# ThatRedox/ChunkyClPlugin

Measured on AMD Instinct MI355X. Metric: Msamples/s, 32x32-chunk scene @1920x1080, higher is better.
Workload: dtype f32

## Files before the change

### chunkyclplugin_amd/csrc/path_state.hpp

```cpp
#pragma once
#include <hip/hip_runtime.h>

#include "kernels.hpp"
#include "rt_device.hpp"

namespace chunky {

struct LdsStack {
    int* base;
    int stride;
    DEV void push(int slot, int v) { base[slot * stride] = v; }
    DEV int pop(int slot) { return base[slot * stride]; }
};
template <int TREE>
DEV void leaf_lookup(const SceneView& S, int bx, int by, int bz, int& data, int& level, int& kind, bool inside = true, int* entry = nullptr) {
    if (TREE < 16 && !inside) bx = by = bz = 0;
    if (TREE == 0) {
        const int* __restrict__ tree = S.octree;
        level = S.octree_depth;
        data = tree[0];
        while (data > 0) {
            level--;
            data = tree[data + ((((bx >> level) & 1) << 2) | (((by >> level) & 1) << 1) | ((bz >> level) & 1))];
        }
// ... 169 lines not shown
    const int sb = i / kSubBlock, px = i % kSubBlock;
    const int x = (bx << kTileLog) + (sb % (kTileEdge / kSubW)) * kSubW + px % kSubW,
              y = (by << kTileLog) + (sb / (kTileEdge / kSubW)) * kSubH + px / kSubW;
    return (x < width && y < height) ? y * width + x : width * height;
}
DEV unsigned fast_quotient(unsigned n, FastDiv f) { return f.m ? __umulhi(n, f.m) >> f.s : n; }

struct SlotPixel {
    int gid, x, y;
};
DEV SlotPixel pool_slot_pixel(const ShardView& T, int width, int height, int slot, FastDiv by_bw) {
    if (T.world != 1 && T.tile != 0) {
        const int gid = slot < T.n_local ? shard_gid(T, slot) : width * height;
        return SlotPixel{gid, gid % width, gid / width};
    }
    const int bw = (width + kTileEdge - 1) >> kTileLog;
    int b = slot >> (2 * kTileLog);
    const int i = slot & (kSampleTile - 1);
    if (T.world != 1) {
        b = b * T.world + T.rank;
        if (b >= bw * ((height + kTileEdge - 1) >> kTileLog)) return SlotPixel{width * height, 0, 0};
    }
    const int by = (int)fast_quotient((unsigned)b, by_bw), bx = b - by * bw;
    const int sb = i / kSubBlock, px = i % kSubBlock;
    const int x = (bx << kTileLog) + (sb % (kTileEdge / kSubW)) * kSubW + px % kSubW,
              y = (by << kTileLog) + (sb / (kTileEdge / kSubW)) * kSubH + px / kSubW;
    return SlotPixel{(x < width && y < height) ? y * width + x : width * height, x, y};
}
__host__ __device__ inline long long pool_tiles(const ShardView& T, int width, int height) {
    if (T.world != 1) return ((long long)T.n_local + kSampleTile - 1) / kSampleTile;
    return (long long)((width + kTileEdge - 1) >> kTileLog) * ((height + kTileEdge - 1) >> kTileLog);
}
DEV int count_lanes(bool p) { return (int)__builtin_popcountll(__ballot(p)); }
enum : int {
    ST_MARCH = 0, ST_BLOCK = 1, ST_SHADE = 2,
    ST_MODEL = 6,
    ST_BVH = 9,
    ST_LEAF = 11,
    ST_TRACED = 10,
    ST_DONE = 3,
    ST_NEXT = 4,
    ST_SETUP = 5,
    ST_IDLE = 7,
    ST_START = 8
};

struct LaneState {
    int gid;
    int sidx;
    unsigned pass : 8;
    unsigned slot : 1;
    unsigned serial : 23;
    f3 mean;
    unsigned rng;
    f3 radiance, throughput, o, d;
    unsigned depth : 8;
    unsigned shadow : 1;
    unsigned oct_hit : 1;
    unsigned trace_hit : 1;
    unsigned cand_level : 4;
    unsigned bvh_which : 1;
    f3 inv;
    float dist_march;
    int steps;
    int cand_data;
    int bvh_cur;
    int bvh_top;
    const int* bvh_base;
    int bvh_head;
    float bvh_dist;
    f3 far;
    int pid;
    unsigned tkind : 2;
    unsigned after_nee : 1;
    f3 pend;
    Hit h;
};

DEV int floor_to_int(float x) {
    int r;
    asm("v_cvt_flr_i32_f32 %0, %1" : "=v"(r) : "v"(x));
    return r;
}

template <bool GUARD = true>
DEV float leaf_exit_distance(const LaneState& L, f3 far, f3 po, int bx, int by, int bz, int level) {
    const int keep = -1 << level;
    const float size = __builtin_ldexpf(1.0f, level);
    const float x0 = (float)(bx & keep), y0 = (float)(by & keep), z0 = (float)(bz & keep);
    float tx = (rt_fma(far.x, size, x0) - po.x) * L.inv.x, ty = (rt_fma(far.y, size, y0) - po.y) * L.inv.y, tz = (rt_fma(far.z, size, z0) - po.z) * L.inv.z;
    if (GUARD) {
        tx = rt_fmax(tx, -rt_inf());
        ty = rt_fmax(ty, -rt_inf());
        tz = rt_fmax(tz, -rt_inf());
    }
    return rt_fmin(tx, rt_fmin(ty, tz));
}
DEV f3 far_of(const f3& inv) { return mk3(inv.x > 0 ? 1.0f : 0.0f, inv.y > 0 ? 1.0f : 0.0f, inv.z > 0 ? 1.0f : 0.0f); }

template <int TREE, bool FARREG = true>
DEV void leaf_exit(const SceneView& S, LaneState& L, f3 po, int bx, int by, int bz, int level) {
    L.dist_march += leaf_exit_distance(L, FARREG ? L.far : far_of(L.inv), po, bx, by, bz, level) + kOffset;
    L.steps += 1;
}

template <int END, bool FARREG = true>
DEV int trace_setup(const SceneView& S, LaneState& L) {
    const int depth = S.octree_depth;
    L.inv = rcp3(L.d);
    if (FARREG) L.far = far_of(L.inv);
    L.dist_march = 0;
    L.steps = 0;
    L.oct_hit = false;
    int lx = (int)rt_floor(L.o.x) >> depth, ly = (int)rt_floor(L.o.y) >> depth, lz = (int)rt_floor(L.o.z) >> depth;
    if ((lx != 0) | (ly != 0) | (lz != 0)) {
        float size = (float)(1 << depth);
        float dist = box_quick(0, size, 0, size, 0, size, L.o, L.inv);
        if (dist != dist || dist < 0) return END;
        L.dist_march += dist + kOffset;
    }
    return ST_MARCH;
}

typedef unsigned long long LaneMask;
DEV bool in_mask(LaneMask m) { return __builtin_amdgcn_inverse_ballot_w64(m); }

DEV unsigned world_edge(const SceneView& S) {
    unsigned edge = 1u << S.octree_depth;
    asm("" : "+s"(edge));
    return edge;
}
template <int TREE, bool GUARD = true>
DEV void march_step(const SceneView& S, const RenderOpts& O, LaneState& L, LaneMask marching, LaneMask& cand_out,
                    LaneMask& live_out, int& data, int& level, const unsigned edge, const LaneMask* far_masks = nullptr, int* entry = nullptr) {
    f3 pos = L.o + L.d * L.dist_march;
    f3 po = pos + L.d * kOffset;
    int bx = floor_to_int(po.x), by = floor_to_int(po.y), bz = floor_to_int(po.z);
    const bool inside = (unsigned)(bx | by | bz) < edge;
    const LaneMask live = marching & __ballot(L.steps < O.draw_depth) & __ballot(!(L.dist_march > L.h.distance)) & __ballot(inside);
    int kind;
    leaf_lookup<TREE>(S, bx, by, bz, data, level, kind, inside, entry);
    const LaneMask hittable = __ballot(kind < 2);
    const LaneMask cand = live & hittable, go = live & ~hittable;
    const f3 far = far_masks ? mk3(in_mask(far_masks[0]) ? 1.0f : 0.0f, in_mask(far_masks[1]) ? 1.0f : 0.0f, in_mask(far_masks[2]) ? 1.0f : 0.0f)
                             : L.far;
    const float step = leaf_exit_distance<GUARD>(L, far, po, bx, by, bz, level) + kOffset;
    const bool advance = in_mask(go);
    L.dist_march = advance ? L.dist_march + step : L.dist_march;
    asm("v_addc_co_u32_e64 %0, vcc, 0, %0, %1" : "+v"(L.steps) : "s"(go) : "vcc");
    cand_out = cand;
    live_out = live;
}

template <int TREE, int END, bool FARREG = true, int KINDS = kBlockAny>
DEV int block_phase(const SceneView& S, LaneState& L) {
    f3 pos = L.o + L.d * L.dist_march;
    f3 po = pos + L.d * kOffset;
    int bx = (int)rt_floor(po.x), by = (int)rt_floor(po.y), bz = (int)rt_floor(po.z);
    Hit t = L.h;
    float dist = block_hit<KINDS>(S, L.cand_data, bx, by, bz, pos, L.d, L.inv, t);
    if (!L.shadow) {
        L.h.normal = t.normal;
        L.h.color = t.color;
        L.h.emittance = t.emittance;
        L.h.spec = t.spec;
    }
    if (dist == dist) {
        if (!L.shadow) {
            L.h.distance = L.dist_march + dist;
            L.h.material = L.cand_data;
        }
        L.oct_hit = true;
        return END;
    }
    leaf_exit<TREE, FARREG>(S, L, po, bx, by, bz, L.cand_level);
    return ST_MARCH;
}
struct WorkQueue {
    int* next;
};
struct WaveArgs {
    SceneView S;
    CameraView C;
    RenderOpts O;
    ShardView T;
    PassSeeds P;
    WorkQueue Q;
    float* res;
    unsigned long long* stats;
    unsigned stack_bytes;
    float* staging;
    unsigned n_samples;
    unsigned xcd_stripe;
    FastDiv div_sub;
    FastDiv div_bw;
    const int* seeds_dev;
};
static_assert(sizeof(WaveArgs) <= 4096, "launch arguments must fit the 4 KB kernel-argument segment");
typedef const WaveArgs __attribute__((address_space(4))) * WaveArgPtr;

template <typename T>
DEV T arg_copy(const T __attribute__((address_space(4))) * p) {
#if defined(__HIP_DEVICE_COMPILE__)
    return *p;
#else
    (void)p;
    return T{};
#endif
}

DEV WaveArgPtr fresh_args() {
    WaveArgPtr a = (WaveArgPtr)__builtin_amdgcn_kernarg_segment_ptr();
    asm volatile("" : "+s"(a));
    return a;
}

struct PartTimers {
    unsigned long long t[10];
    unsigned long long last;
};
enum : int { PT_SKY = 0, PT_SAMPLING, PT_SETUP, PT_DEPOSIT, PT_FOLD, PT_OPEN, PT_HANDOUT, PT_NEWSAMPLE };
template <bool ON>
DEV void part_begin(PartTimers* pt) {
    if (ON) pt->last = __builtin_amdgcn_s_memtime();
}
template <bool ON>
DEV void part_end(PartTimers* pt, int which) {
    if (ON) {
        const unsigned long long now = __builtin_amdgcn_s_memtime();
        pt->t[which] += now - pt->last;
        pt->last = now;
    }
}

template <int TREE, bool BVH, bool PROF = false>
DEV int shade_phase(const SceneView& S, const RenderOpts& O, LaneState& L, LdsStack& stack, PartTimers* pt = nullptr) {
    part_begin<PROF>(pt);
    const bool hit = BVH ? L.trace_hit : L.oct_hit;
    const bool main_trace = !L.shadow;
    if (!hit) {
        const float e = main_trace ? 1.0f : rt_fabs(dot(L.d, L.h.normal));
        L.radiance = L.radiance + sky_radiance(S, L.d, L.throughput, e);
    }
    part_end<PROF>(pt, PT_SKY);
    bool finished = !hit && main_trace;
    bool to_sun = false;
    if (finished) {
    } else if (main_trace) {
        L.o = L.o + L.d * (L.h.distance - kOffset);
        f3 c = mk3(L.h.color.x, L.h.color.y, L.h.color.z);
        L.throughput = L.throughput * c;
        L.radiance = L.radiance + (c * (L.h.emittance * O.emitter_scale)) * L.throughput;
        if (S.sun_flags & 1) to_sun = true;
    } else {
        L.shadow = false;
    }
    if (!finished) {
        const float x1 = rt_pcg_float(&L.rng), x2 = rt_pcg_float(&L.rng);
        float sn, cs;
        rt_sincos(2 * RT_PI_F * x2, &sn, &cs);
        const float cos_a = 1 - x1 + x1 * S.sun_radius_cos;
        const float root = rt_sqrt(to_sun ? 1 - cos_a * cos_a : x1);
        const f3 n = L.h.normal;
        f3 a;
        float len2;
        if (to_sun) {
            const f3 u = S.su * (cs * root), v = S.sv * (sn * root), w = S.sw * cos_a;
            a = (u * v) + w;
            len2 = dot(a, a);
        } else {
            float xx, xy, xz = 0;
            if ((double)rt_fabs(n.x) > 0.1) {
                xx = 0;
                xy = 1;
            } else {
                xx = 1;
                xy = 0;
            }
            a = mk3(xy * n.z - xz * n.y, xz * n.x - xx * n.z, xx * n.y - xy * n.x);
            len2 = a.x * a.x + a.y * a.y + a.z * a.z;
        }
        const float rl = 1 / rt_sqrt(len2);
        a = a * rl;
        if (to_sun) {
            L.d = a;
            L.shadow = true;
        } else {
            const float tx = root * cs, ty = root * sn, tz = rt_sqrt(1 - x1);
            const float vx = a.y * n.z - a.z * n.y, vy = a.z * n.x - a.x * n.z, vz = a.x * n.y - a.y * n.x;
            L.d = f3{a.x * tx + vx * ty + n.x * tz, a.y * tx + vy * ty + n.y * tz, a.z * tx + vz * ty + n.z * tz};
            L.o = L.o + L.d * kOffset;
            L.depth += 1;
            L.h.distance = rt_inf();
            finished = !(L.depth < O.max_depth);
        }
    }
    part_end<PROF>(pt, PT_SAMPLING);
    return finished ? ST_NEXT : ST_SETUP;
}

DEV f3 cosine_direction(f3 n, float x1, float x2) {
    float r = rt_sqrt(x1);
    float theta = 2 * RT_PI_F * x2;
    float st, ct;
    rt_sincos(theta, &st, &ct);
    float tx = r * ct, ty = r * st, tz = rt_sqrt(1 - x1);
    float xx, xy, xz = 0;
    if ((double)rt_fabs(n.x) > 0.1) {
        xx = 0;
        xy = 1;
    } else {
// ... 42 lines not shown
```

### chunkyclplugin_amd/csrc/pool_kernel.inc

```
template <int TREE, int K, bool STATS, bool BVH = false, bool EXT = false, bool SORT = false>
__global__ void __launch_bounds__(256, ((STATS || EXT) ? 4 : (BVH ? CHUNKY_POOL_BVH_WAVES : CHUNKY_POOL_WAVES))) render_pool(WaveArgs unused_by_name) {
    constexpr int WORDS = EXT ? 9 : (BVH ? 8 : CHUNKY_POOL_WORDS);
    constexpr int END = BVH ? ST_TRACED : ST_SHADE;
    constexpr bool SPLIT = SORT;
    static_assert(!SORT || (TREE != 0 && !BVH && !EXT), "sorted block tests: the plain kernel on the re-laid-out tree only");
    extern __shared__ int lds[];
    const int lane = (int)(threadIdx.x & 63u), wave = (int)(threadIdx.x >> 6);
    PoolLds P{nullptr, nullptr, nullptr};
    PathStacks stacks{nullptr, 64 + K};
    {
        const unsigned depth = BVH ? fresh_args()->stack_bytes : 0u;
        char* base = (char*)lds + wave * (K * 16 * WORDS + K * 8 + (64 + K) * depth * 4);
        P.park = (uint4*)base;
        P.tags = (int*)(base + K * 16 * WORDS);
        P.list = P.tags + K;
        stacks.base = (int*)(base + K * 16 * WORDS + K * 8);
        if (lane < K) P.park[lane] = make_uint4(0u, 0u, kFreshDepth | (WORDS <= 7 ? 0u : (unsigned)(64 + lane) << 16), 0u);
    }
    LdsStack stack{lds, 0};
    LaneState L;
    L.h.material = 0;
    L.h.normal = mk3(0, 0, 0);
    L.h.color = f4{0, 0, 0, 0};
    L.h.emittance = 0;
    L.h.distance = 0;
    L.cand_data = 0;
    L.cand_level = 0;
    L.pass = 0;
    L.gid = -1;
    L.sidx = 0;
    L.pid = lane;
    L.tkind = 0;
    L.after_nee = false;
    L.pend = mk3(0, 0, 0);
    L.h.spec = 0;
    L.mean = mk3(0, 0, 0);
    L.slot = 0;
    L.serial = 0;
    L.steps = 0;
    L.rng = 0;
    L.depth = kFreshDepth;
    L.shadow = false;
    L.dist_march = 0;
    L.radiance = mk3(0, 0, 0);
    L.throughput = mk3(0, 0, 0);
    L.o = L.d = L.inv = L.far = mk3(0, 0, 0);
    L.oct_hit = false;
    L.trace_hit = false;
    L.bvh_cur = L.bvh_top = L.bvh_which = L.bvh_head = 0;
    L.bvh_base = nullptr;
    L.bvh_dist = 0;
    unsigned long long prof[9] = {0, 0, 0, 0, 0, 0, 0, 0, 0};
    unsigned long long swap_rounds = 0, swapped = 0;
    PartTimers parts{{0, 0, 0, 0, 0, 0, 0, 0, 0, 0}, 0};
    unsigned long long t_begin = 0;
    if (STATS) t_begin = __builtin_amdgcn_s_memtime();
    XcdClaim claim{xcd_first_range(), 0u, 0u};
    int ranges_tried = 0;
    int st = ST_SHADE;
    int ptag = lane < K ? ST_SHADE : ST_DONE;
    wave_lds_fence();
    int c_march = 0, c_block = 0, c_shade = 0, c_bvh = 0, c_leaf = 0, c_model = 0;
    int model_age = 0;
    auto census = [&]() {
        if (BVH && __ballot(st == ST_TRACED)) {
            const SceneView S = arg_copy(&fresh_args()->S);
            if (st == ST_TRACED) st = rbvh_begin(S, L);
        }
        c_march = count_lanes(st == ST_MARCH) + count_lanes(ptag == ST_MARCH);
        c_block = count_lanes(st == ST_BLOCK) + count_lanes(ptag == ST_BLOCK);
        c_shade = count_lanes(st == ST_SHADE) + count_lanes(ptag == ST_SHADE);
        c_model = SPLIT ? count_lanes(st == ST_MODEL) + count_lanes(ptag == ST_MODEL) : 0;
        c_bvh = BVH ? count_lanes(st == ST_BVH) + count_lanes(ptag == ST_BVH) : 0;
        c_leaf = BVH ? count_lanes(st == ST_LEAF) + count_lanes(ptag == ST_LEAF) : 0;
    };
    census();
    while ((c_march | c_block | c_shade | c_bvh | c_leaf | c_model) != 0) {
        const int v_march = (c_march < 64 ? c_march : 64) * kWMarch, v_block = (c_block < 64 ? c_block : 64) * kWBlock,
                  v_shade = (c_shade < 64 ? c_shade : 64) * kWShade;
        int X = (int)((unsigned)(v_march - v_block - 1) >> 31);
        int v_best = v_block > v_march ? v_block : v_march;
        if (v_shade >= v_best) {
            X = 2;
            v_best = v_shade;
        }
        if (SPLIT) {
            const int v_model = (c_model < 64 ? c_model : 64) * kWModel;
            model_age += 1;
            if (v_model > v_best || c_model * model_age >= kModelFire) {
                X = ST_MODEL;
                v_best = v_model > v_best ? v_model : v_best;
                model_age = 0;
            }
        }
        if (BVH) {
            const int c_walk = c_bvh + c_leaf;
            const int v_walk = (c_walk < 64 ? c_walk : 64) * kWWalk;
            if (v_walk > v_best) { X = 5; v_best = v_walk; }
        }
        unsigned long long t0 = 0;
        if (STATS) t0 = __builtin_amdgcn_s_memtime();
        if (K > 0) {
            const int n = pool_swap<K, WORDS>(P, L, st, ptag, X, lane);
            if (STATS && n) {
                swap_rounds += 1;
                swapped += (unsigned long long)n;
            }
        }
        if (STATS) {
            parts.t[PT_FOLD] += __builtin_amdgcn_s_memtime() - t0;
            parts.t[PT_OPEN] += 1;
            parts.t[PT_HANDOUT] += X == 0 ? 1 : 0;
        }
        int n_exec = 0;
        if (X == 0) {
            WaveArgPtr A = fresh_args();
            const SceneView Sm = arg_copy(&A->S);
            const RenderOpts Om = arg_copy(&A->O);
            const LaneMask entered = __ballot(st == ST_MARCH);
            int nm = __popcll(entered);
            n_exec = nm;
            const int parked_march = c_march - nm;
            const int other_b = c_block < 64 ? c_block : 64, other_s = c_shade < 64 ? c_shade : 64;
            int other = other_b > other_s ? other_b : other_s;
            if (SPLIT) {
                const int other_m = c_model < 64 ? c_model : 64;
                other = other > other_m ? other : other_m;
            }
            int stay = (other + nm + 1) >> 1;
            if (parked_march < kStayFewParked) stay -= BVH ? kStayLongerBvh : kStayLonger;
            if (K > 0 && parked_march >= kPoolRefill && stay < 65 - kPoolRefill) stay = 65 - kPoolRefill;
            if (stay < 1) stay = 1;
            LaneMask marching = entered, to_block = 0;
            L.far = far_of(L.inv);
            const LaneMask* far_masks = nullptr;
            int data, level, entry = 0;
            const float ninf = -rt_inf();
            const bool guard = ((__ballot(L.inv.x == ninf) | __ballot(L.inv.y == ninf) | __ballot(L.inv.z == ninf)) & entered) != 0;
            if (guard)
                march_loop<TREE, true, STATS>(Sm, Om, L, marching, to_block, data, level, nm, stay, far_masks, prof, SPLIT ? &entry : nullptr);
            else
                march_loop<TREE, false, STATS>(Sm, Om, L, marching, to_block, data, level, nm, stay, far_masks, prof, SPLIT ? &entry : nullptr);
            const bool found = in_mask(to_block);
            L.cand_data = found ? data : L.cand_data;
            L.cand_level = found ? level : L.cand_level;
            const int st_found = SPLIT && (entry & 0x2000000) ? ST_MODEL : ST_BLOCK;
            st = found ? st_found : (in_mask(entered & ~marching & ~to_block) ? END : st);
            if (STATS) {
                prof[0] -= 1;
                prof[1] -= (unsigned long long)n_exec;
            }
        } else if (X == 1) {
            n_exec = count_lanes(st == ST_BLOCK);
            const SceneView S = arg_copy(&fresh_args()->S);
            if (st == ST_BLOCK) {
                st = block_phase<TREE, END, false, SPLIT ? kBlockCubes : kBlockAny>(S, L);
                if (WORDS == 6 && st == END) hit_to_march_registers(L);
            }
        } else if (SPLIT && X == ST_MODEL) {
            n_exec = count_lanes(st == ST_MODEL);
            if (STATS) parts.t[8] += (unsigned long long)n_exec + (1ull << 40);
            const SceneView S = arg_copy(&fresh_args()->S);
            asm volatile("; chunky-mark models");
            if (st == ST_MODEL) {
                st = block_phase<TREE, END, false, kBlockModels>(S, L);
                if (WORDS == 6 && st == END) hit_to_march_registers(L);
            }
            asm volatile("; chunky-mark models-end");
        } else if (BVH && X == 5) {
            const SceneView S = arg_copy(&fresh_args()->S);
            int nw = count_lanes(st == ST_BVH);
            n_exec = nw;
            const int parked_walk = c_bvh + c_leaf - nw;
            int stay = nw - kWalkLeave + 1;
            if (K > 0 && parked_walk > 0) {
                const int refill = parked_walk < kWalkLeave ? parked_walk : kWalkLeave;
                if (stay < 65 - refill) stay = 65 - refill;
            }
            if (stay < 1) stay = 1;
            do {
                if (STATS) {
                    prof[3] += 1;
                    prof[4] += (unsigned long long)nw;
                }
                if (st == ST_BVH) st = rwalk_step(S, L, stacks);
                nw = count_lanes(st == ST_BVH);
            } while (nw >= stay);
            if (STATS) {
                prof[3] -= 1;
                prof[4] -= (unsigned long long)n_exec;
            }
        } else {
            n_exec = count_lanes(st == ST_SHADE);
            WaveArgPtr A = fresh_args();
            const SceneView S = arg_copy(&A->S);
            const RenderOpts O = arg_copy(&A->O);
            const bool served = st == ST_SHADE;
            bool fresh = served && L.depth == kFreshDepth;
            if (served && !fresh) {
                if (WORDS == 6) march_registers_to_hit(L);
                st = EXT ? shade_phase_ext<TREE, BVH>(S, O, L) : shade_phase<TREE, BVH, STATS>(S, O, L, stack, &parts);
            }
            part_begin<STATS>(&parts);
            if (st == ST_NEXT) {
                float* __restrict__ out = A->staging + 3 * (size_t)(unsigned)L.sidx;
#if CHUNKY_STAGING_STORE == 1
                out[0] = L.radiance.x, out[1] = L.radiance.y, out[2] = L.radiance.z;
#elif CHUNKY_STAGING_STORE == 2
                __hip_atomic_store(out, L.radiance.x, __ATOMIC_RELAXED, __HIP_MEMORY_SCOPE_AGENT);
                __hip_atomic_store(out + 1, L.radiance.y, __ATOMIC_RELAXED, __HIP_MEMORY_SCOPE_AGENT);
                __hip_atomic_store(out + 2, L.radiance.z, __ATOMIC_RELAXED, __HIP_MEMORY_SCOPE_AGENT);
#elif CHUNKY_STAGING_STORE == 3
                __hip_atomic_store(out, L.radiance.x, __ATOMIC_RELAXED, __HIP_MEMORY_SCOPE_SYSTEM);
                __hip_atomic_store(out + 1, L.radiance.y, __ATOMIC_RELAXED, __HIP_MEMORY_SCOPE_SYSTEM);
                __hip_atomic_store(out + 2, L.radiance.z, __ATOMIC_RELAXED, __HIP_MEMORY_SCOPE_SYSTEM);
#else
                __builtin_nontemporal_store(L.radiance.x, out);
                __builtin_nontemporal_store(L.radiance.y, out + 1);
                __builtin_nontemporal_store(L.radiance.z, out + 2);
#endif
                fresh = true;
            }
            part_end<STATS>(&parts, PT_DEPOSIT);
            const bool need = fresh;
            const unsigned sidx = xcd_claim(A->Q.next + kXcdCounters, claim, ranges_tried, need, A->xcd_stripe, A->n_samples);
            if (need && sidx != kClaimNone) {
                const unsigned n_samples = A->n_samples;
                if (sidx >= n_samples) {
                    st = ST_DONE;
                    fresh = false;
                } else {
                    const CameraView C = arg_copy(&A->C);
                    const ShardView T = arg_copy(&A->T);
                    const unsigned per_sub = (unsigned)A->P.n * (unsigned)kSubBlock;
                    const unsigned sub = fast_quotient(sidx, arg_copy(&A->div_sub)), rem = sidx - sub * per_sub;
                    const unsigned pass = rem / (unsigned)kSubBlock;
                    const int slot = (int)(sub * (unsigned)kSubBlock + (rem & (unsigned)(kSubBlock - 1)));
                    const SlotPixel px = pool_slot_pixel(T, C.width, C.height, slot, arg_copy(&A->div_bw));
                    const int gid = px.gid;
                    if (gid < C.width * C.height) {
                        const int* seeds_dev = A->seeds_dev;
                        const unsigned seed = (unsigned)(seeds_dev ? seeds_dev[pass] : A->P.seed[pass]);
                        unsigned rng = seed + (unsigned)gid;
                        rt_pcg_next(&rng);
                        const RayOD pr = primary_ray<CHUNKY_POOL_PROJ>(C, seed, gid, rng, false, px.x, px.y);
                        L.sidx = (int)sidx;
                        L.rng = rng;
                        L.o = pr.o;
                        L.d = pr.d;
                        L.radiance = mk3(0, 0, 0);
                        L.throughput = mk3(1, 1, 1);
                        L.depth = 0;
                        L.shadow = false;
                        L.tkind = 0;
                        L.after_nee = false;
                        L.h.distance = rt_inf();
                        st = ST_SETUP;
                        fresh = false;
                    }
                }
            }
            part_end<STATS>(&parts, PT_NEWSAMPLE);
            if (fresh) {
                st = ST_SHADE;
                L.depth = kFreshDepth;
            }
            if (st == ST_SETUP) st = trace_setup<END, false>(S, L);
            part_end<STATS>(&parts, PT_SETUP);
        }
        if (STATS) {
            const unsigned long long dt = __builtin_amdgcn_s_memtime() - t0;
#pragma unroll
            for (int k = 0; k < 3; k++)
                if (X == k) {
                    prof[3 * k] += 1;
                    prof[3 * k + 1] += (unsigned long long)n_exec;
                    prof[3 * k + 2] += dt;
                }
            if (X == ST_MODEL) parts.t[9] += dt;
            if (X == 5) {
                prof[3] += 1;
                prof[4] += (unsigned long long)n_exec;
                prof[5] += dt;
            }
        }
        census();
    }
    if (STATS && lane == 0) {
        unsigned long long* stats = fresh_args()->stats;
        for (int k = 0; k < 9; k++) atomicAdd(&stats[k], prof[k]);
        const unsigned long long life = __builtin_amdgcn_s_memtime() - t_begin;
        atomicAdd(&stats[9], life);
        atomicMax(&stats[10], life);
        atomicAdd(&stats[11], 1ull);
        atomicAdd(&stats[12], swap_rounds);
        atomicAdd(&stats[13], swapped);
        for (int k = 0; k < 10; k++) atomicAdd(&stats[14 + k], parts.t[k]);
    }
}
```

### chunkyclplugin_amd/csrc/render_pool.hip

```cpp
#include <hip/hip_runtime.h>

#include <cstdlib>

#include "path_state.hpp"
#include "pool_walk.hpp"

#ifndef CHUNKY_STAGING_STORE
#define CHUNKY_STAGING_STORE 0
#endif

namespace chunky {

template <int TREE, bool BVH>
DEV int shade_phase_ext(const SceneView& S, const RenderOpts& O, LaneState& L) {
    const bool hit = BVH ? L.trace_hit : L.oct_hit;
    const int kind = L.tkind;
    const f3 n = L.h.normal;
    int next = 0;
    if (kind == 0) {
        if (!hit) {
            L.radiance = L.radiance + sky_radiance(S, L.d, L.throughput, 1.0f);
            return ST_NEXT;
        }
        const f3 d_in = L.d;
// ... 26 lines not shown
            L.o = L.o + refl * kOffset;
            next = 4;
        } else {
            L.throughput = thr_d;
            next = 1;
        }
    } else if (kind == 1) {
        if (!hit) L.radiance = L.radiance + sky_radiance(S, L.d, L.throughput, L.h.emittance);
        next = 2;
    } else {
        if (!hit) L.radiance = L.radiance + L.pend;
        next = 3;
    }
    if (next == 1) {
        const bool sun_on = O.sun_sampling < 0 ? (S.sun_flags & 1) != 0 : O.sun_sampling != 0;
        if (sun_on) {
            L.d = sun_sample(S, L.rng);
            L.h.emittance = rt_fabs(dot(L.d, n));
            L.tkind = 1;
            L.shadow = true;
            return ST_SETUP;
        }
        next = 2;
    }
    if (next == 2) {
        next = 3;
        if (O.nee && O.emitters && S.n_emitters > 0 && (int)L.depth + 1 < O.max_depth) {
            const float xk = rt_pcg_float(&L.rng), xf = rt_pcg_float(&L.rng), xu = rt_pcg_float(&L.rng), xv = rt_pcg_float(&L.rng);
            int k = (int)(xk * (float)S.n_emitters);
            if (k > S.n_emitters - 1) k = S.n_emitters - 1;
            int face = (int)(xf * 6.0f);
            if (face > 5) face = 5;
            const int4 em = S.emitters[k];
            const int level = (em.w >> 25) & 15, block = em.w & 0x1FFFFFF;
            const float size = (float)(1 << level);
            const float a = xu * size, b = xv * size;
            const float fa = a - rt_floor(a), fb = b - rt_floor(b);
            const float ex = (float)em.x, ey = (float)em.y, ez = (float)em.z;
            f3 pe, nf;
            float tu, tv;
            switch (face) {
                case 0: pe = mk3(ex, ey + a, ez + b); nf = mk3(-1, 0, 0); tu = 1 - fb; tv = fa; break;
                case 1: pe = mk3(ex + size, ey + a, ez + b); nf = mk3(1, 0, 0); tu = fb; tv = fa; break;
                case 2: pe = mk3(ex + a, ey, ez + b); nf = mk3(0, -1, 0); tu = fa; tv = 1 - fb; break;
                case 3: pe = mk3(ex + a, ey + size, ez + b); nf = mk3(0, 1, 0); tu = fa; tv = fb; break;
                case 4: pe = mk3(ex + a, ey + b, ez); nf = mk3(0, 0, -1); tu = fa; tv = fb; break;
                default: pe = mk3(ex + a, ey + b, ez + size); nf = mk3(0, 0, 1); tu = 1 - fa; tv = fb; break;
            }
            const f3 l = pe - L.o;
            const float d2 = dot(l, l);
            const float dist = rt_sqrt(d2);
            const f3 dir = l * (1 / dist);
            const float cs = dot(dir, n), cl = -dot(dir, nf);
            L.after_nee = true;
            if (cs > 0 && cl > 0 && dist > 0.002f) {
                Hit er = L.h;
                if (material_sample(S, S.blocks[block + 1], tu, tv, er) && er.emittance > 0) {
                    const float w = (cs * cl) / (RT_PI_F * d2) * (6.0f * (float)S.n_emitters * (size * size));
                    const f3 ce = mk3(er.color.x, er.color.y, er.color.z);
                    const f3 le = ce * (ce * (er.emittance * O.emitter_scale));
                    L.pend = L.throughput * (le * w);
                    L.d = dir;
                    L.h.distance = dist - 0.001f;
                    L.tkind = 2;
                    L.shadow = true;
                    return ST_SETUP;
                }
            }
        }
    }
    if (next == 3) {
        const float x1 = rt_pcg_float(&L.rng), x2 = rt_pcg_float(&L.rng);
        L.d = cosine_direction(n, x1, x2);
        L.o = L.o + L.d * kOffset;
    }
    L.depth += 1;
    L.h.distance = rt_inf();
    L.tkind = 0;
    L.shadow = false;
    return (int)L.depth < O.max_depth ? ST_SETUP : ST_NEXT;
}
constexpr unsigned kFreshDepth = 255u;

struct PoolLds {
    uint4* park;
    int* tags;
    int* list;
};

template <bool BVH>
DEV int phase_class(int st) {
    return BVH && st >= ST_BVH ? 5 : st;
}

template <int WORDS>
DEV void pool_pack(const LaneState& L, uint4 (&v)[WORDS]) {
    constexpr bool SHORT = WORDS <= 7;
    constexpr int H = SHORT ? 5 : 6;
    const unsigned misc = (unsigned)L.depth | ((unsigned)L.shadow << 8) | ((unsigned)L.oct_hit << 9) | ((unsigned)L.trace_hit << 10) |
                          ((unsigned)L.cand_level << 11) | ((unsigned)L.bvh_which << 15) |
                          (SHORT ? (unsigned)L.steps << 16 : ((unsigned)L.pid << 16) | ((unsigned)L.tkind << 24) | ((unsigned)L.after_nee << 26));
    if (WORDS > 8) v[WORDS - 1] = make_uint4(__float_as_uint(L.pend.x), __float_as_uint(L.pend.y), __float_as_uint(L.pend.z), (unsigned)L.h.spec);
    v[0] = make_uint4((unsigned)L.sidx, L.rng, misc, SHORT ? (unsigned)L.cand_data : (unsigned)L.steps);
    v[1] = make_uint4(__float_as_uint(L.radiance.x), __float_as_uint(L.radiance.y), __float_as_uint(L.radiance.z), __float_as_uint(L.throughput.x));
    v[2] = make_uint4(__float_as_uint(L.throughput.y), __float_as_uint(L.throughput.z), __float_as_uint(L.o.x), __float_as_uint(L.o.y));
    v[3] = make_uint4(__float_as_uint(L.o.z), __float_as_uint(L.d.x), __float_as_uint(L.d.y), __float_as_uint(L.d.z));
    if (WORDS == 6) {
        v[4] = make_uint4(__float_as_uint(L.inv.x), __float_as_uint(L.inv.y), __float_as_uint(L.inv.z), __float_as_uint(L.dist_march));
        v[5] = make_uint4(__float_as_uint(L.h.distance), __float_as_uint(L.h.normal.x), __float_as_uint(L.h.normal.y), __float_as_uint(L.h.normal.z));
        return;
    }
    v[4] = make_uint4(__float_as_uint(L.inv.x), __float_as_uint(L.inv.y), __float_as_uint(L.inv.z), __float_as_uint(L.dist_march));
    if (WORDS > 7) v[5] = make_uint4((unsigned)L.bvh_cur, (unsigned)L.bvh_top, __float_as_uint(L.bvh_dist), (unsigned)L.cand_data);
    v[H] = make_uint4(__float_as_uint(L.h.distance), __float_as_uint(L.h.normal.x), __float_as_uint(L.h.normal.y), __float_as_uint(L.h.normal.z));
    v[H + 1] = make_uint4(__float_as_uint(L.h.color.x), __float_as_uint(L.h.color.y), __float_as_uint(L.h.color.z), __float_as_uint(L.h.emittance));
}
template <int WORDS>
DEV void pool_unpack(LaneState& L, const uint4 (&v)[WORDS]) {
    constexpr bool SHORT = WORDS <= 7;
    constexpr int H = SHORT ? 5 : 6;
    if (WORDS > 8) {
        L.pend = mk3(__uint_as_float(v[WORDS - 1].x), __uint_as_float(v[WORDS - 1].y), __uint_as_float(v[WORDS - 1].z));
        L.h.spec = (int)v[WORDS - 1].w;
    }
    L.sidx = (int)v[0].x; L.rng = v[0].y;
    L.depth = v[0].z & 0xFFu; L.shadow = (v[0].z >> 8) & 1u; L.oct_hit = (v[0].z >> 9) & 1u; L.trace_hit = (v[0].z >> 10) & 1u;
    L.cand_level = (v[0].z >> 11) & 15u; L.bvh_which = (v[0].z >> 15) & 1u;
    if (SHORT) {
        L.steps = (int)(v[0].z >> 16);
        L.cand_data = (int)v[0].w;
    } else {
        L.pid = (int)((v[0].z >> 16) & 0xFFu); L.tkind = (v[0].z >> 24) & 3u; L.after_nee = (v[0].z >> 26) & 1u;
        L.steps = (int)v[0].w;
        L.bvh_cur = (int)v[5].x; L.bvh_top = (int)v[5].y; L.bvh_dist = __uint_as_float(v[5].z);
        L.cand_data = (int)v[5].w;
    }
    L.radiance = mk3(__uint_as_float(v[1].x), __uint_as_float(v[1].y), __uint_as_float(v[1].z));
    L.throughput = mk3(__uint_as_float(v[1].w), __uint_as_float(v[2].x), __uint_as_float(v[2].y));
    L.o = mk3(__uint_as_float(v[2].z), __uint_as_float(v[2].w), __uint_as_float(v[3].x));
    L.d = mk3(__uint_as_float(v[3].y), __uint_as_float(v[3].z), __uint_as_float(v[3].w));
    L.inv = mk3(__uint_as_float(v[4].x), __uint_as_float(v[4].y), __uint_as_float(v[4].z));
    L.dist_march = __uint_as_float(v[4].w);
    if (WORDS == 6) {
        L.h.distance = __uint_as_float(v[5].x);
        L.h.normal = mk3(__uint_as_float(v[5].y), __uint_as_float(v[5].z), __uint_as_float(v[5].w));
        return;
    }
    L.h.distance = __uint_as_float(v[H].x);
    L.h.normal = mk3(__uint_as_float(v[H].y), __uint_as_float(v[H].z), __uint_as_float(v[H].w));
    L.h.color = f4{__uint_as_float(v[H + 1].x), __uint_as_float(v[H + 1].y), __uint_as_float(v[H + 1].z), 0.0f};
    L.h.emittance = __uint_as_float(v[H + 1].w);
}

DEV void hit_to_march_registers(LaneState& L) {
    L.inv = mk3(L.h.color.x, L.h.color.y, L.h.color.z);
    L.dist_march = L.h.emittance;
}
DEV void march_registers_to_hit(LaneState& L) {
    L.h.color = f4{L.inv.x, L.inv.y, L.inv.z, 0.0f};
    L.h.emittance = L.dist_march;
}

DEV void wave_lds_fence() {
    __builtin_amdgcn_fence(__ATOMIC_RELEASE, "wavefront");
    __builtin_amdgcn_wave_barrier();
    __builtin_amdgcn_fence(__ATOMIC_ACQUIRE, "wavefront");
}

template <int K, int WORDS = 8>
DEV int pool_swap(PoolLds P, LaneState& L, int& st, int& ptag, int X, int lane) {
    constexpr bool BVH = WORDS == 8 || WORDS == 9;
    constexpr LaneMask kSlots = K >= 64 ? ~0ull : ((1ull << K) - 1ull);
    const LaneMask m_done = __ballot(st == ST_DONE);
    const LaneMask m_goes = __ballot(phase_class<BVH>(st) != X);
    const LaneMask m_in = __ballot(phase_class<BVH>(ptag) == X) & kSlots;
    const int n_out = (int)__popcll(m_goes), n_in = (int)__popcll(m_in);
    const int n = n_out < n_in ? n_out : n_in;
    if (n == 0) return 0;
    const int r_in = (int)__builtin_amdgcn_mbcnt_hi((unsigned)(m_in >> 32), __builtin_amdgcn_mbcnt_lo((unsigned)m_in, 0u));
    int r_out;
    if (m_done == 0) {
        r_out = (int)__builtin_amdgcn_mbcnt_hi((unsigned)(m_goes >> 32), __builtin_amdgcn_mbcnt_lo((unsigned)m_goes, 0u));
    } else {
        const bool done = st == ST_DONE;
        const LaneMask m_mine = done ? m_done : (m_goes & ~m_done);
        r_out = (done ? 0 : (int)__popcll(m_done)) + (int)__builtin_amdgcn_mbcnt_hi((unsigned)(m_mine >> 32), __builtin_amdgcn_mbcnt_lo((unsigned)m_mine, 0u));
    }
    const bool comes = in_mask(m_in) && r_in < n, goes = in_mask(m_goes) && r_out < n;
    if (comes) P.list[r_in] = lane | (ptag << 8);
    if (goes) P.tags[r_out] = st;
    wave_lds_fence();
    if (comes) ptag = P.tags[r_in];
    if (goes) {
        const int e = P.list[r_out];
        const int s = e & 0xFF;
        uint4 mine[WORDS], theirs[WORDS];
        pool_pack<WORDS>(L, mine);
#pragma unroll
        for (int g = 0; g < WORDS; g++) {
            unsigned long long* q = (unsigned long long*)&P.park[g * K + s];
            const unsigned long long lo = __hip_atomic_exchange(q, (unsigned long long)mine[g].x | ((unsigned long long)mine[g].y << 32), __ATOMIC_RELAXED, __HIP_MEMORY_SCOPE_WAVEFRONT);
            const unsigned long long hi = __hip_atomic_exchange(q + 1, (unsigned long long)mine[g].z | ((unsigned long long)mine[g].w << 32), __ATOMIC_RELAXED, __HIP_MEMORY_SCOPE_WAVEFRONT);
            theirs[g] = make_uint4((unsigned)lo, (unsigned)(lo >> 32), (unsigned)hi, (unsigned)(hi >> 32));
        }
        st = e >> 8;
        pool_unpack<WORDS>(L, theirs);
    }
    wave_lds_fence();
    return n;
}
#ifndef CHUNKY_POOL_WAVES
#define CHUNKY_POOL_WAVES 6
#endif
#ifndef CHUNKY_POOL_BVH_WAVES
#define CHUNKY_POOL_BVH_WAVES 5
#endif
#ifndef CHUNKY_POOL_WORDS
#define CHUNKY_POOL_WORDS 6
#endif
#ifndef CHUNKY_POOL_PARK
#define CHUNKY_POOL_PARK (CHUNKY_POOL_WORDS == 6 ? 64 : 56)
#endif
#ifndef CHUNKY_POOL_REFILL
#define CHUNKY_POOL_REFILL 20
#endif
#ifndef CHUNKY_WALK_LEAVE
#define CHUNKY_WALK_LEAVE 24
#endif
#ifndef CHUNKY_STAY_FEW_PARKED
#define CHUNKY_STAY_FEW_PARKED 12
#endif
#ifndef CHUNKY_STAY_LONGER
#define CHUNKY_STAY_LONGER 16
#endif
constexpr int kPoolPark = CHUNKY_POOL_PARK, kPoolRefill = CHUNKY_POOL_REFILL, kWalkLeave = CHUNKY_WALK_LEAVE;
#ifndef CHUNKY_STAY_LONGER_BVH
#define CHUNKY_STAY_LONGER_BVH 6
#endif
constexpr int kStayFewParked = CHUNKY_STAY_FEW_PARKED, kStayLonger = CHUNKY_STAY_LONGER, kStayLongerBvh = CHUNKY_STAY_LONGER_BVH;
#ifndef CHUNKY_W_MODEL
#define CHUNKY_W_MODEL 4
#endif
#ifndef CHUNKY_MODEL_FIRE
#define CHUNKY_MODEL_FIRE 560
#endif
constexpr int kWModel = CHUNKY_W_MODEL, kModelFire = CHUNKY_MODEL_FIRE;
constexpr int kWWalk = 1;
constexpr int kSampleBatch = 256;

constexpr int kXcdRanges = 8;
constexpr int kXcdCounters = 64;
DEV int xcd_id() {
    unsigned x;
    asm volatile("s_getreg_b32 %0, hwreg(HW_REG_XCC_ID)" : "=s"(x));
    return (int)(x & 7u);
}
DEV int xcd_first_range() { return xcd_id(); }
struct XcdClaim {
    int q;
    unsigned next, end;
};
DEV unsigned xcd_range_size(unsigned x, unsigned stripe, unsigned n_samples) {
    const unsigned lo = x * stripe;
    return lo >= n_samples ? 0u : (n_samples - lo < stripe ? n_samples - lo : stripe);
}
constexpr unsigned kClaimNone = 0xFFFFFFFEu, kClaimDone = 0xFFFFFFFFu;
DEV unsigned xcd_claim(int* counters, XcdClaim& c, int& tried, bool need, unsigned stripe, unsigned n_samples) {
    const unsigned long long mask = __ballot(need);
    if (mask == 0) return kClaimNone;
    const unsigned n_need = (unsigned)__popcll(mask);
    const unsigned rank = __builtin_amdgcn_mbcnt_hi((unsigned)(mask >> 32), __builtin_amdgcn_mbcnt_lo((unsigned)mask, 0u));
    const unsigned rem = c.end - c.next;
    unsigned sidx = kClaimNone;
    if (need && rank < rem) sidx = c.next + rank;
    c.next += n_need < rem ? n_need : rem;
    if (n_need > rem) {
        bool got = false;
        while (tried < kXcdRanges) {
            int b = 0;
            if (need && rank == 0) b = atomicAdd(counters + c.q, kSampleBatch);
            const unsigned base = (unsigned)__builtin_amdgcn_readfirstlane(__shfl(b, __ffsll((long long)mask) - 1));
            const unsigned n_q = xcd_range_size((unsigned)c.q, stripe, n_samples);
            if (base < n_q) {
                c.next = (unsigned)c.q * stripe + base;
                c.end = c.next + (n_q - base < (unsigned)kSampleBatch ? n_q - base : (unsigned)kSampleBatch);
                got = true;
                break;
            }
            c.q = c.q + 1 == kXcdRanges ? 0 : c.q + 1;
            tried += 1;
        }
        if (!got) {
            if (need && rank >= rem) sidx = kClaimDone;
            c.next = c.end = 0u;
        } else {
            const unsigned mine = c.next + (rank - rem);
            if (need && rank >= rem && mine < c.end) sidx = mine;
            c.next = c.next + (n_need - rem) < c.end ? c.next + (n_need - rem) : c.end;
        }
    }
    return sidx;
}

template <int TREE, bool GUARD, bool STATS>
DEV void march_loop(const SceneView& Sm, const RenderOpts& Om, LaneState& L, LaneMask& marching, LaneMask& to_block, int& data, int& level,
                    int& nm, int stay, const LaneMask* far_masks, unsigned long long* prof, int* entry = nullptr) {
    const unsigned edge = world_edge(Sm);
    do {
        if (STATS) {
            prof[0] += 1;
            prof[1] += (unsigned long long)nm;
        }
        LaneMask cand, live;
        march_step<TREE, GUARD>(Sm, Om, L, marching, cand, live, data, level, edge, far_masks, entry);
        to_block |= cand;
        marching = live & ~cand;
        nm = __popcll(marching);
    } while (nm >= stay);
}

#define CHUNKY_POOL_PROJ false
#include "pool_kernel.inc"
#undef CHUNKY_POOL_PROJ
namespace proj {
#define CHUNKY_POOL_PROJ true
#include "pool_kernel.inc"
#undef CHUNKY_POOL_PROJ
}
template <int TREE, int K, bool STATS, bool BVH = false, bool EXT = false, bool SORT = false>
static void (*pool_kernel(bool projected))(WaveArgs) {
    return projected ? proj::render_pool<TREE, K, STATS, BVH, EXT, SORT> : render_pool<TREE, K, STATS, BVH, EXT, SORT>;
}

__global__ void __launch_bounds__(256) fold_kernel(const float* __restrict__ staging, float* __restrict__ res, ShardView T, int n_pixels,
                                                    int width, long long n_slots, int n_passes, int first_spp) {
    const long long t = (long long)blockIdx.x * 256 + threadIdx.x;
    if (t >= 3ll * n_slots) return;
    const int slot = (int)(t / 3), c = (int)(t - 3ll * slot);
    const int gid = pool_slot_gid(T, width, n_pixels / width, slot);
    if (gid >= n_pixels) return;
    float mean = res[3 * (size_t)gid + c];
    const size_t sub = (size_t)slot / kSubBlock, i = (size_t)slot % kSubBlock;
    const float* p = staging + 3 * (sub * (size_t)n_passes * kSubBlock + i) + c;
#pragma unroll 8
    for (int k = 0; k < n_passes; k++) {
        const int spp = first_spp + k;
        mean = (mean * (float)spp + p[(size_t)k * (3 * kSubBlock)]) / (float)(spp + 1);
    }
    res[3 * (size_t)gid + c] = mean;
}

template <bool PACK>
__global__ void __launch_bounds__(256) gather_kernel(ShardView T, int width, int height, float* __restrict__ fb, float* __restrict__ packed) {
    const int slot = (int)(blockIdx.x * 256 + threadIdx.x);
    if (slot >= T.n_local) return;
    const int gid = pool_slot_gid(T, width, height, slot);
    if (gid >= width * height) return;
    float* a = fb + 3 * (size_t)gid;
    float* b = packed + 3 * (size_t)slot;
    if (PACK) {
        b[0] = a[0]; b[1] = a[1]; b[2] = a[2];
    } else {
        a[0] = b[0]; a[1] = b[1]; a[2] = b[2];
    }
}
__global__ void __launch_bounds__(256) clear_foreign_kernel(ShardView T, int width, int height, float* __restrict__ fb) {
    const int gid = (int)(blockIdx.x * 256 + threadIdx.x);
    if (gid >= width * height || T.world == 1) return;
    int unit;
    if (T.tile != 0) {
        unit = gid / T.tile;
    } else {
        const int y = gid / width, x = gid - y * width;
        unit = (y >> kTileLog) * ((width + kTileEdge - 1) >> kTileLog) + (x >> kTileLog);
    }
    if (unit % T.world == T.rank) return;
    float* a = fb + 3 * (size_t)gid;
    a[0] = 0.0f; a[1] = 0.0f; a[2] = 0.0f;
}
static hipError_t launch_pool(int variant, const SceneView& S, const CameraView& C, const RenderOpts& O, const ShardView& T,
                              const PassSeeds& P, float* res, int* work_counter, hipStream_t stream, KernelChoice* chosen,
                              float* staging, const int* seeds_dev, float* fold_stats = nullptr) {
    const int block = 256;
    int n_cu = 0;
    if (hipError_t e = current_device_cus(&n_cu)) return e;
    if (T.n_local <= 0 || P.n <= 0) return hipSuccess;
    const bool stats = (variant & 4) != 0;
    int tree = tree_form(variant, S);
    const bool bvh = !S.world_bvh_empty || !S.actor_bvh_empty;
    int depth = 0;
    if (bvh) depth = S.bvh_stack_entries > 0 && S.bvh_stack_entries < kBvhStackEntries ? S.bvh_stack_entries : kBvhStackEntries;
    int park = kPoolPark;
    switch ((variant >> 6) & 3) {
        case 1: park = 0; break;
        case 2: park = 32; break;
        default: break;
    }
    typedef void (*Kernel)(WaveArgs);
    Kernel k;
    const bool proj = C.projector_type > 0;
    const bool ext = opts_extended(O);
    const bool sorted = ((variant & 256) || S.sort_blocks) && !(variant & 512) && !bvh && !ext && tree != 0 && S.block_info != nullptr;
    bool sorted_ran = false;
    int words = bvh ? 8 : CHUNKY_POOL_WORDS;
    if (ext) {
        if (tree != 17 && tree != 18) tree = -1;
        words = 9;
        park = bvh ? 16 : 32;
        if (bvh)
            k = tree == 17 ? pool_kernel<17, 16, false, true, true>(proj) : (tree == 18 ? pool_kernel<18, 16, false, true, true>(proj) : pool_kernel<-1, 16, false, true, true>(proj));
        else
            k = tree == 17 ? pool_kernel<17, 32, false, false, true>(proj) : (tree == 18 ? pool_kernel<18, 32, false, false, true>(proj) : pool_kernel<-1, 32, false, false, true>(proj));
    } else if (bvh) {
        if (tree != 17 && tree != 18) tree = -1;
        park = 5 * 4 * (32 * 136 + (64 + 32) * depth * 4) <= 160 * 1024 ? 32 : 16;
        if (stats) {
            if (tree != 17) tree = -1;
            park = 16;
            k = tree == 17 ? pool_kernel<17, 16, true, true>(proj) : pool_kernel<-1, 16, true, true>(proj);
#ifdef CHUNKY_POOL_BVH_PARK
        } else if (true) {
            if (tree != 17) tree = -1;
            park = CHUNKY_POOL_BVH_PARK;
            k = tree == 17 ? pool_kernel<17, CHUNKY_POOL_BVH_PARK, false, true>(proj) : pool_kernel<-1, CHUNKY_POOL_BVH_PARK, false, true>(proj);
#endif
        } else if (park == 32) {
            k = tree == 17 ? pool_kernel<17, 32, false, true>(proj) : (tree == 18 ? pool_kernel<18, 32, false, true>(proj) : pool_kernel<-1, 32, false, true>(proj));
        } else {
            k = tree == 17 ? pool_kernel<17, 16, false, true>(proj) : (tree == 18 ? pool_kernel<18, 16, false, true>(proj) : pool_kernel<-1, 16, false, true>(proj));
        }
    } else if (stats) {
        if (tree != 17) tree = -1;
        park = kPoolPark;
        if (sorted) k = tree == 17 ? pool_kernel<17, kPoolPark, true, false, false, true>(proj) : pool_kernel<-1, kPoolPark, true, false, false, true>(proj);
        else k = tree == 17 ? pool_kernel<17, kPoolPark, true>(proj) : pool_kernel<-1, kPoolPark, true>(proj);
        sorted_ran = sorted;
    } else if (park != kPoolPark) {
        if (tree != 0) tree = -1;
        if (park == 0) k = tree == 0 ? pool_kernel<0, 0, false>(proj) : pool_kernel<-1, 0, false>(proj);
        else k = tree == 0 ? pool_kernel<0, 32, false>(proj) : pool_kernel<-1, 32, false>(proj);
    } else if (sorted) {
        switch (tree) {
            case 16: k = pool_kernel<16, kPoolPark, false, false, false, true>(proj); break;
            case 17: k = pool_kernel<17, kPoolPark, false, false, false, true>(proj); break;
            case 18: k = pool_kernel<18, kPoolPark, false, false, false, true>(proj); break;
            case 19: k = pool_kernel<19, kPoolPark, false, false, false, true>(proj); break;
            default: tree = -1; k = pool_kernel<-1, kPoolPark, false, false, false, true>(proj); break;
        }
        sorted_ran = true;
    } else {
        switch (tree) {
            case 0: k = pool_kernel<0, kPoolPark, false>(proj); break;
            case 16: k = pool_kernel<16, kPoolPark, false>(proj); break;
            case 17: k = pool_kernel<17, kPoolPark, false>(proj); break;
            case 18: k = pool_kernel<18, kPoolPark, false>(proj); break;
            case 19: k = pool_kernel<19, kPoolPark, false>(proj); break;
            default: tree = -1; k = pool_kernel<-1, kPoolPark, false>(proj); break;
        }
    }
    size_t lds = (size_t)(block / 64) * (size_t)(park * 16 * words + park * 8 + (64 + park) * depth * 4);
    int occ = 0;
    hipError_t e = hipOccupancyMaxActiveBlocksPerMultiprocessor(&occ, k, block, lds);
    if (e != hipSuccess) return e;
    const int bpc = occ > 0 ? occ : 1;
    const long long n_tiles = pool_tiles(T, C.width, C.height);
    const long long n_samples = n_tiles * kSampleTile * P.n;
    const long long want = (n_samples + (long long)(block / 64) * (64 + park) - 1) / ((long long)(block / 64) * (64 + park));
    int grid = n_cu * bpc;
    if ((long long)grid > want) grid = (int)want;
    if (chosen) *chosen = KernelChoice{tree, 1, bvh ? 1 : 0, grid, park, ext ? 1 : 0, sorted_ran ? 1 : 0};
    e = hipMemsetAsync(work_counter, 0, sizeof(int), stream);
    if (e != hipSuccess) return e;
// ... 65 lines not shown
```

Baseline: 7665.

## Share hit-color registers with march state in block phase and split phase branches

Adds a SHARE variant of block_phase for the 6-word pool layout that writes hit color and emittance directly into the inv and dist_march registers. This removes the separate Hit copy and the hit_to_march_registers step. The phase dispatch changes from an if/else chain to independent if blocks, each followed by an inline-asm marker that ties X to an SGPR. That is likely meant to keep the compiler from merging register live ranges across phases. The extra asm barriers could limit scheduling, and the branch conversion relies on X selecting exactly one phase.

```diff
diff --git a/chunkyclplugin_amd/csrc/path_state.hpp b/chunkyclplugin_amd/csrc/path_state.hpp
--- a/chunkyclplugin_amd/csrc/path_state.hpp
+++ b/chunkyclplugin_amd/csrc/path_state.hpp
@@ -345,11 +345,29 @@
     live_out = live;
 }
 
-template <int TREE, int END, bool FARREG = true, int KINDS = kBlockAny>
+template <int TREE, int END, bool FARREG = true, int KINDS = kBlockAny, bool SHARE = false>
 DEV int block_phase(const SceneView& S, LaneState& L) {
     f3 pos = L.o + L.d * L.dist_march;
     f3 po = pos + L.d * kOffset;
     int bx = (int)rt_floor(po.x), by = (int)rt_floor(po.y), bz = (int)rt_floor(po.z);
+    if (SHARE) {
+        Hit t;
+        t.normal = L.h.normal;
+        const float dist = block_hit<KINDS>(S, L.cand_data, bx, by, bz, pos, L.d, L.inv, t);
+        if (!L.shadow) L.h.normal = t.normal;
+        if (dist == dist) {
+            if (!L.shadow) {
+                L.h.distance = L.dist_march + dist;
+                L.h.material = L.cand_data;
+            }
+            L.inv = mk3(t.color.x, t.color.y, t.color.z);
+            L.dist_march = t.emittance;
+            L.oct_hit = true;
+            return END;
+        }
+        leaf_exit<TREE, FARREG>(S, L, po, bx, by, bz, L.cand_level);
+        return ST_MARCH;
+    }
     Hit t = L.h;
     float dist = block_hit<KINDS>(S, L.cand_data, bx, by, bz, pos, L.d, L.inv, t);
     if (!L.shadow) {
diff --git a/chunkyclplugin_amd/csrc/pool_kernel.inc b/chunkyclplugin_amd/csrc/pool_kernel.inc
--- a/chunkyclplugin_amd/csrc/pool_kernel.inc
+++ b/chunkyclplugin_amd/csrc/pool_kernel.inc
@@ -150,24 +150,28 @@
                 prof[0] -= 1;
                 prof[1] -= (unsigned long long)n_exec;
             }
-        } else if (X == 1) {
+        }
+        CHUNKY_PHASE_END(X, "march");
+        if (X == 1) {
             n_exec = count_lanes(st == ST_BLOCK);
             const SceneView S = arg_copy(&fresh_args()->S);
             if (st == ST_BLOCK) {
-                st = block_phase<TREE, END, false, SPLIT ? kBlockCubes : kBlockAny>(S, L);
-                if (WORDS == 6 && st == END) hit_to_march_registers(L);
-            }
-        } else if (SPLIT && X == ST_MODEL) {
+                st = block_phase<TREE, END, false, SPLIT ? kBlockCubes : kBlockAny, WORDS == 6>(S, L);
+            }
+        }
+        CHUNKY_PHASE_END(X, "block");
+        if (SPLIT && X == ST_MODEL) {
             n_exec = count_lanes(st == ST_MODEL);
             if (STATS) parts.t[8] += (unsigned long long)n_exec + (1ull << 40);
             const SceneView S = arg_copy(&fresh_args()->S);
             asm volatile("; chunky-mark models");
             if (st == ST_MODEL) {
-                st = block_phase<TREE, END, false, kBlockModels>(S, L);
-                if (WORDS == 6 && st == END) hit_to_march_registers(L);
+                st = block_phase<TREE, END, false, kBlockModels, WORDS == 6>(S, L);
             }
             asm volatile("; chunky-mark models-end");
-        } else if (BVH && X == 5) {
+        }
+        CHUNKY_PHASE_END(X, "model-blocks");
+        if (BVH && X == 5) {
             const SceneView S = arg_copy(&fresh_args()->S);
             int nw = count_lanes(st == ST_BVH);
             n_exec = nw;
@@ -190,7 +194,9 @@
                 prof[3] -= 1;
                 prof[4] -= (unsigned long long)n_exec;
             }
-        } else {
+        }
+        CHUNKY_PHASE_END(X, "walk");
+        if (X == 2) {
             n_exec = count_lanes(st == ST_SHADE);
             WaveArgPtr A = fresh_args();
             const SceneView S = arg_copy(&A->S);
@@ -268,6 +274,7 @@
             if (st == ST_SETUP) st = trace_setup<END, false>(S, L);
             part_end<STATS>(&parts, PT_SETUP);
         }
+        CHUNKY_PHASE_END(X, "shade");
         if (STATS) {
             const unsigned long long dt = __builtin_amdgcn_s_memtime() - t0;
 #pragma unroll
diff --git a/chunkyclplugin_amd/csrc/render_pool.hip b/chunkyclplugin_amd/csrc/render_pool.hip
--- a/chunkyclplugin_amd/csrc/render_pool.hip
+++ b/chunkyclplugin_amd/csrc/render_pool.hip
@@ -202,10 +202,6 @@
     L.h.emittance = __uint_as_float(v[H + 1].w);
 }
 
-DEV void hit_to_march_registers(LaneState& L) {
-    L.inv = mk3(L.h.color.x, L.h.color.y, L.h.color.z);
-    L.dist_march = L.h.emittance;
-}
 DEV void march_registers_to_hit(LaneState& L) {
     L.h.color = f4{L.inv.x, L.inv.y, L.inv.z, 0.0f};
     L.h.emittance = L.dist_march;
@@ -368,6 +364,8 @@
         nm = __popcll(marching);
     } while (nm >= stay);
 }
+
+#define CHUNKY_PHASE_END(X, name) asm volatile("; chunky-mark phase-end " name : "+s"(X))
 
 #define CHUNKY_POOL_PROJ false
 #include "pool_kernel.inc"
```

Measured after the change: 7894 (median of 6 runs). 1.03x the previous value.
